# junqiangchen/PytorchDeepLearing

Hardware: AMD Instinct MI355X
Metric: volumes/sec VNet3d 96^3 fp16 train step (higher is better)
Workload: dtype f16; 1 GPU; VNet3d(1,1) binary seg, 4x1x96^3 per GPU, BinaryDiceLoss + Dice metric, AdamW, dropout p=0.2 on, random-init weights (BASELINE.json configs[2]); global_batch=4, parallelism=dp1, loss_semantics=per-rank (DDP)

## Files before the change

### include/segengine.h

```cpp
#ifndef SEGENGINE_H
#define SEGENGINE_H
#ifdef __cplusplus
extern "C" {
#endif

typedef struct seg_engine* seg_handle;

enum { SEG_NET_VNET = 0, SEG_NET_UNET = 1, SEG_NET_RESNET = 2 };
enum { SEG_F32 = 0, SEG_F16 = 1, SEG_BF16 = 2 };
enum { SEG_LABEL_U8 = 0, SEG_LABEL_I32 = 1, SEG_LABEL_I64 = 2, SEG_LABEL_F32 = 3,
       SEG_LABEL_BINARIZE = 16 };
enum {
    SEG_LOSS_BINARY_DICE = 0,
    SEG_LOSS_BINARY_CE = 1,
    SEG_LOSS_BINARY_FOCAL = 2,
    SEG_LOSS_BINARY_CE_DICE = 3,
    SEG_LOSS_MULTI_CE = 4,
    SEG_LOSS_MULTI_FOCAL = 5,
    SEG_LOSS_MULTI_DICE = 6,
    SEG_LOSS_BINARY_JACCARD = 7,
    SEG_LOSS_BINARY_ELDICE = 8,
    SEG_LOSS_BINARY_TVERSKY = 9,
    SEG_LOSS_MULTI_CE_DICE = 10,
    SEG_LOSS_MULTI_ELDICE = 11,
// ... 130 lines not shown
    int Cout, Ngemm, K, Kpad;
    int sd, sh, sw;
    int scatter;
    seg_taps taps;
    const float* act_scale;
    const float* act_shift;
    void* out1;
    int Cout0;
    const void* rq_r;
    const float* rq_scale;
    const float* rq_shift;
    double* rq_Q;
} seg_conv_args;
int seg_op_conv(const seg_conv_args* a, int dtype, void* stream);
int seg_op_conv_kernel(const seg_conv_args* a);

typedef struct seg_wgrad_args {
    const void* dr;
    const void* x0;
    const void* x1;
    int C0, C1;
    float* dw;
    int P, Q;
    int N, ID, IH, IW, OD, OH, OW;
    int sd, sh, sw;
    seg_taps taps;
    long long sP, sQ, sT;
    int stem;
    const float* act_scale;
    const float* act_shift;
} seg_wgrad_args;
long long seg_op_wgrad_partial_bytes(const seg_wgrad_args* a);
int seg_op_wgrad(const seg_wgrad_args* a, float* partial_scratch, int dtype, void* stream);

typedef struct seg_pack_desc {
    const float* src;
    void* dst;
    int R1, R2, T, Cc;
    int Kpad;
    long long s1, s2, sT, sC;
    int flipT;
    int csrc;
    int frag;
} seg_pack_desc;
int seg_op_pack(const seg_pack_desc* descs, int ndesc, long long max_elems, int dtype, void* stream);
int seg_op_conv3(const void* in, const void* w, const float* bias, void* out, double* stats, int n, int d, int h,
                 int wid, int cin, int cout, int ndim, int dtype, void* stream);
long long seg_op_wgrad3_partial_bytes(int ndim, int n, int d, int h, int wid, int p, int q);
int seg_op_wgrad3(const void* dr, const void* x, float* partial, float* dw, int n, int d, int h, int wid, int p,
                  int q, int ndim, int dtype, void* stream);
int seg_op_wgrad3_cat(const void* dr, const void* x0, const void* x1, int c0, float* partial, float* dw, int n, int d, int h,
                      int wid, int p, int q, int ndim, int dtype, void* stream);
typedef struct seg_stemx_args {
    const void* img; const void* w3; const void* w1;
    const float* bias3; const float* bias1;
    double* stats3; double* stats1;
    const float* scale3; const float* shift3; const float* scale1; const float* shift1;
    void* out;
    const void* dy[3]; int ndy;
    double* Q3; double* Q1;
    const float* coef3; const float* coef1;
    float* partial;
    int N, D, H, W, Cimg;
} seg_stemx_args;
long long seg_op_stemx_partial_bytes(int ndim, int n, int d, int h, int wid, int cimg);
long long seg_op_stemx_moment_bytes(int ndim, int n, int d, int h, int wid, int cimg);
// ... 135 lines not shown
```

### pytorchdeeplearing_amd/_capi.py

```python
import ctypes as C
import os

HERE = os.path.dirname(os.path.abspath(__file__))
LIB_PATH = os.environ.get("SEGENGINE_LIB") or os.path.join(HERE, "lib", "libsegengine.so")

NET_KIND = {"vnet": 0, "unet": 1, "resnet": 2}
DTYPE = {"f32": 0, "fp32": 0, "float32": 0, "f16": 1, "fp16": 1, "float16": 1, "bf16": 2, "bfloat16": 2}
LABEL_TYPES = {"torch.uint8": 0, "torch.int32": 1, "torch.int64": 2, "torch.float32": 3}
LOSS_KIND = {
    "BinaryDiceLoss": 0, "BinaryCrossEntropyLoss": 1, "BinaryFocalLoss": 2, "BinaryCrossEntropyDiceLoss": 3,
    "MutilCrossEntropyLoss": 4, "MutilFocalLoss": 5, "MutilDiceLoss": 6,
    "BinaryJaccardLoss": 7, "BinaryELDiceLoss": 8, "BinaryTverskyLoss": 9, "MutilCrossEntropyDiceLoss": 10, "MutilELDiceLoss": 11, "BinarySSLoss": 12,
    "MutilTverskyLoss": 13, "MutilSSLoss": 14, "MCC_Loss": 15,
}
LABEL_BINARIZE = 16
MASKS_EVAL, MASKS_GIVEN, MASKS_RANDOM = 0, 1, 2


def label_type(t, binarize=False):
    return LABEL_TYPES[str(t.dtype)] | (LABEL_BINARIZE if binarize else 0)
KERNEL_CLASSES = ["conv3", "wgrad3", "conv_generic", "wgrad_generic", "stem", "gn_act", "gn_bwd_reduce", "gn_bwd_apply", "head", "conv3_smallbox", "gn_group", "misc", "cls_head"]

_vp, _i, _ll, _f, _d = C.c_void_p, C.c_int, C.c_longlong, C.c_float, C.c_double

# ... 19 lines not shown
    "seg_backward_bucket": (_i, [_vp, C.c_double, C.POINTER(C.c_int), C.POINTER(C.c_longlong)]),
    "seg_backward_range": (_i, [_vp, _vp, _i, _i, _i, _vp]),
    "seg_backward_slice": (_i, [_vp, _vp, _i, _i, _i, _i, _vp]),
    "seg_side_wait": (_i, [_vp, _vp]),
    "seg_feature_find": (_i, [_vp, C.c_char_p, C.POINTER(_i), C.POINTER(_i)]),
    "seg_feature_read": (_i, [_vp, _i, _i, _vp, _vp]),
    "seg_gradcam_ws_bytes": (_ll, [_vp, _i]),
    "seg_gradcam": (_i, [_vp, C.POINTER(_i), _i, _vp, _vp, _vp]),
    "seg_set_loss_scale": (_i, [_vp, _f]),
    "seg_get_loss_scale": (_f, [_vp]),
    "seg_loss_ws_bytes": (_ll, [_i, _i]),
    "seg_loss_forward": (_i, [_vp, _vp, _i, _i, _i, _ll, _i, _f, _f, _vp, _vp, _vp, _vp]),
    "seg_loss_shared_doubles": (_i, []),
    "seg_loss_reduce": (_i, [_vp, _vp, _i, _i, _i, _ll, _i, _f, _f, _vp, _vp]),
    "seg_loss_finalize": (_i, [_vp, _vp, _i, _i, _i, _ll, _i, _f, _f, _vp, _i, _vp, _vp, _vp]),
    "seg_loss_backward": (_i, [_vp, _vp, _i, _i, _i, _ll, _i, _f, _f, _vp, _f, _vp, _vp]),
    "seg_lovasz_ws_bytes": (_ll, [_i, _ll]),
    "seg_lovasz_forward": (_i, [_vp, _vp, _i, _i, _i, _ll, _vp, _vp, _vp, _vp]),
    "seg_ssim_ws_bytes": (_ll, [_i, _i, _ll]),
    "seg_ssim_forward": (_i, [_vp, _vp, _i, _i, _i, _i, _i, _i, _i, _vp, _vp, _vp]),
    "seg_ssim_forward_cols": (_i, [_vp, _vp, _i, _i, _i, _i, _i, _i, _i, _vp, _vp, _vp, _vp]),
    "seg_ssim_backward": (_i, [_vp, _vp, _i, _i, _i, _i, _i, _i, _i, _vp, _vp, _i, _vp, _vp, _vp]),
    "seg_predict_mask": (_i, [_vp, _vp, _i, _i, _ll, C.c_float, _i, _vp]),
    "seg_metric": (_i, [_vp, _vp, _i, _i, _i, _ll, _vp, _vp, _vp]),
    "seg_train_step": (_i, [_vp, _vp, _vp]),
    "seg_train_graph_capture": (_i, [_vp, _vp, _vp]),
    "seg_train_graph_launch": (_i, [_vp, _vp]),
    "seg_train_graph_ready": (_i, [_vp]),
    "seg_adam_step": (_i, [_vp, _vp, _vp, _vp, _ll, _f, _f, _f, _f, _f, _i, _f, _i, _vp, _vp]),
    "seg_op_conv": (_i, [_vp, _i, _vp]),
    "seg_op_conv_kernel": (_i, [_vp]),
    "seg_op_wgrad": (_i, [_vp, _vp, _i, _vp]),
    "seg_op_wgrad_partial_bytes": (_ll, [_vp]),
    "seg_op_pack": (_i, [_vp, _i, _ll, _i, _vp]),
    "seg_op_conv3": (_i, [_vp, _vp, _vp, _vp, _vp, _i, _i, _i, _i, _i, _i, _i, _i, _vp]),
    "seg_op_conv3x": (_i, [_i, _vp, _vp, _i, _vp, _vp, _vp, _vp, _i, _i, _i, _i, _i, _i, _i, _i, _vp]),
    "seg_op_conv3x_num_cfgs": (_i, []),
    "seg_op_conv3x_cfg_info": (_i, [_i, C.POINTER(_i), C.POINTER(_i), C.POINTER(_i), C.POINTER(_i), C.POINTER(_i), C.c_char_p, _i]),
    "seg_op_conv3x_default_cfg": (_i, [_i, _i, _i, _i, _i, _i, _i, _i]),
    "seg_op_conv3x_cfg_frag": (_i, [_i]),
    "seg_op_wgrad3_partial_bytes": (_ll, [_i, _i, _i, _i, _i, _i, _i]),
    "seg_op_wgrad3": (_i, [_vp, _vp, _vp, _vp, _i, _i, _i, _i, _i, _i, _i, _i, _vp]),
    "seg_op_wgrad3_cat": (_i, [_vp, _vp, _vp, _i, _vp, _vp, _i, _i, _i, _i, _i, _i, _i, _i, _vp]),
    "seg_op_stemx_partial_bytes": (_ll, [_i, _i, _i, _i, _i, _i]),
    "seg_op_stemx_moment_bytes": (_ll, [_i, _i, _i, _i, _i, _i]),
    "seg_op_stemx": (_i, [_vp, _i, _i, _i, _vp, _vp, _vp]),
    "seg_abi_sizeof": (_i, [_i]),
    "seg_op_gn_forward": (_i, [_vp, _i, _vp]),
    "seg_op_gn_backward": (_i, [_vp, _i, _vp]),
    "seg_op_gn_backward_head": (_i, [_vp, _vp, _vp, _vp, _i, _vp]),
    "seg_op_gn_coop_plan": (_i, [_i, _ll, _i, _i, C.POINTER(_i), C.POINTER(_i)]),
    "seg_op_gn_group_eligible": (_i, [_i, _ll, _i]),
    "seg_op_maxpool": (_i, [_vp, _vp, _vp, _vp, _i, _i, _i, _i, _i, _i, _i, _i, _i, _i, _vp]),
    "seg_op_cls_head_ws_bytes": (_ll, [_i, _ll]),
    "seg_op_cls_head_ws_offset": (_ll, [_i, _ll, _i]),
    "seg_op_cls_head_forward": (_i, [_vp, _vp, _vp, _vp, _vp, _vp, _vp, _i, _ll, _i, _vp, _i, _vp]),
    "seg_op_cls_head_backward": (_i, [_vp, _vp, _vp, _vp, _vp, _vp, _vp, _vp, _i, _ll, _i, _i, _vp, _i, _vp]),
    "seg_op_gradcam_ws_bytes": (_ll, [_i, _i, _i, _i, _i, _i, _i, _i]),
    "seg_op_gradcam": (_i, [_vp, _vp, _i, _i, _i, _i, _i, _i, _i, _i, _i, _i, _f, _f, _i, _i, _vp, _vp, _vp]),
    "seg_op_pool3": (_i, [_vp, _vp, _i, _i, _i, _i, _i, _i, _vp]),
    "seg_op_skel_iter": (_i, [_vp, _vp, _vp, _i, _i, _i, _i, _i, _vp]),
    "seg_op_skel_iter_bwd": (_i, [_vp, _vp, _vp, _vp, _vp, _i, _i, _i, _i, _i, _vp]),
    "seg_op_skel_update": (_i, [_vp, _vp, _vp, _i, _i, _i, _i, _i, _vp]),
    "seg_op_skel_update_bwd": (_i, [_vp, _vp, _vp, _vp, _vp, _i, _i, _i, _i, _i, _vp]),
    "seg_op_pool3_bwd": (_i, [_vp, _vp, _vp, _i, _i, _i, _i, _i, _i, _vp]),
    "seg_op_plane_dot_scratch_bytes": (_ll, [_i, _ll]),
# ... 109 lines not shown
```

### pytorchdeeplearing_amd/csrc/capi_ops.hip

```cpp
#include <cmath>

#include "engine_internal.h"

#define SEG_OK(what) (hipGetLastError() == hipSuccess ? 0 : fail(what ": launch failed"))

extern "C" {

long long seg_loss_ws_bytes(int n, int c) { return (long long)align_up(loss_sums_count(n, c) * sizeof(double) * STAT_REP); }

}
namespace segi {
int fill_loss(LossArgs& a, const float* logits, const void* target, int label_type, int n, int c, long long v,
                     int loss_kind, float focal_alpha, float focal_gamma, void* ws) {
    if (!logits || !target || !ws) return fail("loss: null pointer");
    if (c < 1 || c > 16) return fail("loss: classes must be 1..16");
    if (loss_kind < 0 || loss_kind >= L_KIND_COUNT) return fail("loss: unknown loss kind");
    const bool binary_kind = loss_kind <= SEG_LOSS_BINARY_CE_DICE || (loss_kind >= L_BIN_JACCARD && loss_kind <= L_BIN_TVERSKY) || loss_kind == L_BIN_SS ||
                             loss_kind == L_BIN_MCC;
    if ((c == 1) != binary_kind) return fail("loss: binary losses need C == 1, multi-class losses C > 1");
    a.logits = logits; a.target = target; a.label_type = label_type; a.N = n; a.C = c; a.V = v; a.kind = loss_kind;
    a.focal_alpha = focal_alpha; a.focal_gamma = focal_gamma; a.class_alpha = nullptr; a.sums = (double*)ws;
    a.out = nullptr; a.dlogits = nullptr; a.grad_scale = 1.f; a.phase = 0; a.n_global = 0;
    return 0;
}
// ... 365 lines not shown
    return SEG_OK("seg_adam_step");
}
}
extern "C" {
int seg_adam_step(float* params, const float* grads, float* exp_avg, float* exp_avg_sq, long long numel, float lr, float beta1,
                  float beta2, float eps, float weight_decay, int decoupled, float inv_scale, int check_finite, int* state, void* stream) {
    return adam_step_impl(params, grads, exp_avg, exp_avg_sq, numel, lr, beta1, beta2, eps, weight_decay, decoupled, inv_scale, check_finite, state,
                          stream, false);
}

int seg_op_conv(const seg_conv_args* a, int dtype, void* stream) {
    if (!a || !a->in0 || !a->w || !a->out) return fail("seg_op_conv: null pointer");
    const int cin = a->C0 + a->C1;
    if (cin < 8 || (cin & (cin - 1)) || a->C0 % 8) return fail("seg_op_conv: channel counts must be powers of two >= 8");
    if (a->Cout % 16 || a->Ngemm % 16 || a->Kpad % 32 || a->Kpad < a->K) return fail("seg_op_conv: bad GEMM extents");
    if ((a->act_scale || a->act_shift) && !(a->act_scale && a->act_shift && conv_uses_stream_kernel(*a)))
        return fail("seg_op_conv: act_scale / act_shift need the streaming kernel (gather form, seg_op_conv_kernel == 1) and come as a pair");
    if (a->rq_Q && !(a->out1 && conv_uses_stream_kernel(*a))) return fail("seg_op_conv: rq_* need out1 / Cout0 on the streaming kernel and all of rq_r, rq_scale, rq_shift");
    if (a->out1 && !conv_uses_stream_kernel(*a)) return fail("seg_op_conv: out1 / Cout0 need the streaming kernel (gather form, no bias / stats, 16-channel tiles in pairs)");
    launch_conv_igemm(*a, dtype, (hipStream_t)stream);
    return SEG_OK("seg_op_conv");
}
int seg_op_conv_kernel(const seg_conv_args* a) { return a ? (conv_uses_stream_kernel(*a) ? 1 : 0) : -1; }
long long seg_op_wgrad_partial_bytes(const seg_wgrad_args* a) { return a ? (long long)wgrad_partial_bytes(*a) : -1; }
int seg_op_wgrad(const seg_wgrad_args* a, float* partial_scratch, int dtype, void* stream) {
    if (!a || !a->dr || !a->x0 || !a->dw || !partial_scratch) return fail("seg_op_wgrad: null pointer");
    if (a->P % 16) return fail("seg_op_wgrad: P must be a multiple of 16");
    if (a->stem ? (a->Q > 32) : (a->Q % 16 != 0)) return fail("seg_op_wgrad: bad Q");
    if ((a->act_scale || a->act_shift) && !(a->act_scale && a->act_shift && dtype != SEG_F32 && wgrad_act_supported(*a)))
        return fail("seg_op_wgrad: act_scale / act_shift need a 1^d stride-1 conv on 16-bit tensors with C0 <= 64 and come as a pair");
    launch_wgrad(*a, partial_scratch, dtype, (hipStream_t)stream);
    return SEG_OK("seg_op_wgrad");
}
int seg_op_pack(const seg_pack_desc* descs, int ndesc, long long max_elems, int dtype, void* stream) {
    if (!descs || ndesc < 1) return fail("seg_op_pack: no descriptors");
    launch_pack(descs, ndesc, (int)max_elems, dtype, (hipStream_t)stream);
    return SEG_OK("seg_op_pack");
}
int seg_op_conv3(const void* in, const void* w, const float* bias, void* out, double* stats, int n, int d, int h, int wid, int cin,
                 int cout, int ndim, int dtype, void* stream) {
    if (!in || !w || !out) return fail("seg_op_conv3: null pointer");
    if (cin < 16 || (cin & (cin - 1)) || cout % 16) return fail("seg_op_conv3: Cin must be a power of two >= 16, Cout a multiple of 16");
    launch_conv3(in, w, bias, out, stats, n, ndim == 3 ? d : 1, h, wid, cin, cout, ndim, dtype, (hipStream_t)stream);
    return SEG_OK("seg_op_conv3");
}
int seg_op_conv3x(int cfg, const void* in0, const void* in1, int c0, const void* w, const float* bias, void* out, double* stats, int n, int d,
                  int h, int wid, int cin, int cout, int ndim, int dtype, void* stream) {
    if (!in0 || !w || !out) return fail("seg_op_conv3x: null pointer");
    if (ndim != 2 && ndim != 3) return fail("seg_op_conv3x: ndim must be 2 or 3");
    const int dd = ndim == 3 ? d : 1;
    if (!conv3x_supported(dtype, ndim, n, dd, h, wid, cin, cout, c0, in1 != nullptr))
        return fail("seg_op_conv3x: needs a 16-bit dtype, Cin % 32 == 0 (or Cin == 16 without a concat), Cout % 16 == 0 and tensors below 2 GB per sample");
    if (cfg < 0) cfg = conv3x_pick(ndim, n, dd, h, wid, cin, cout);
    if (cfg < 0 || !launch_conv3x(cfg, in0, in1, c0, w, bias, out, stats, n, dd, h, wid, cin, cout, ndim, dtype, (hipStream_t)stream))
        return fail("seg_op_conv3x: the tiling does not fit this shape");
    return SEG_OK("seg_op_conv3x");
}
int seg_op_conv3x_num_cfgs(void) { return conv3x_num_cfgs(); }
int seg_op_conv3x_cfg_frag(int cfg) { return conv3x_cfg_frag(cfg); }
int seg_op_conv3x_cfg_info(int index, int* id, int* ndim, int* box3, int* bn, int* nres, char* name, int name_cap) {
    const char* nm = nullptr;
    if (conv3x_cfg_info(index, id, ndim, box3, bn, nres, &nm)) return fail("seg_op_conv3x_cfg_info: index out of range");
    if (name && name_cap > 0) snprintf(name, name_cap, "%s", nm);
    return 0;
}
int seg_op_conv3x_default_cfg(int ndim, int n, int d, int h, int wid, int cin, int cout, int dtype) {
// ... 303 lines not shown
```

### pytorchdeeplearing_amd/csrc/kernels.h

```cpp
#pragma once
#include "../../include/segengine.h"
#include "common.h"

namespace seg {

typedef seg_taps Taps;
typedef seg_conv_args ConvArgs;
struct StepRider { int* bump = nullptr; const int* gate = nullptr; int* tally = nullptr; int* clear = nullptr; };
__device__ __forceinline__ void step_rider_run(const StepRider& r) {
    if (r.bump) { if (!(r.gate && *r.gate)) *r.bump += 1; else if (r.tally) *r.tally += 1; }
    if (r.clear) *r.clear = 0;
}
void launch_conv_igemm(const ConvArgs& a, int dtype, hipStream_t s, int stat_rep = STAT_REP);
bool conv_uses_stream_kernel(const ConvArgs& a);

void launch_conv3(const void* in, const void* w, const float* bias, void* out, double* stats, int N, int D, int H, int W, int Cin,
                  int Cout, int ndim, int dtype, hipStream_t s, const void* in1 = nullptr, int C0 = 0);
bool conv3x_supported(int dtype, int ndim, int N, int D, int H, int W, int Cin, int Cout, int C0, bool has_in1);
int conv3x_pick(int ndim, int N, int D, int H, int W, int Cin, int Cout, bool has_in1 = false);
int conv3x_cfg_frag(int cfg);
int conv3x_num_cfgs();
int conv3x_cfg_info(int index, int* id, int* ndim, int* box3, int* bn, int* nres, const char** name);
bool launch_conv3x(int cfg, const void* in0, const void* in1, int C0, const void* w, const float* bias, void* out, double* stats, int N, int D,
                   int H, int W, int Cin, int Cout, int ndim, int dtype, hipStream_t s, int stat_rep = STAT_REP);
// ... 128 lines not shown
    const float* vdl; const float* vw; int vK;    int rep_q;
};
struct GnHeadW { double* sums; float* dw; float* db; };
bool gn_head_w_supported(const GnBwdArgs& a);
void launch_gn_bwd_reduce(const GnBwdArgs& a, int dtype, hipStream_t s, const GnHeadW* hw = nullptr);
struct GnBwdFinArgs;
void launch_gn_bwd_apply(const GnBwdArgs& a, int dtype, hipStream_t s, const GnBwdFinArgs* fa = nullptr, const GnBwdFinArgs* fb = nullptr,
                         const GnHeadW* hw = nullptr);

struct GnBwdFinArgs {
    const double* Q;
    const double* stats;
    const float* gamma;
    const float* mask; int mask_ld;
    const float* mean; const float* rstd;
    float* dgamma; float* dbeta;
    float* dbias;
    float* coef;
    int N, C;
    long long V;
    int rep_q, rep_s;
};
void launch_gn_bwd_finalize(const GnBwdFinArgs& a, hipStream_t s, const GnBwdFinArgs* b = nullptr);
bool gn_bwd_group_eligible(int C, long long V, int esz);
void launch_gn_fwd_group(const GnFinArgs& f, const void* r, const void* res, void* out, int dtype, hipStream_t s);
void launch_gn_bwd_group(const GnBwdArgs& e, const GnBwdFinArgs& f, int dtype, hipStream_t s);
bool gn_bwd_coop_plan(int C, long long V, int N, int esz, int* S, int* ku);
bool gn_bwd_coop_eligible(const GnBwdArgs& e, int esz);
void launch_gn_bwd_coop(const GnBwdArgs& e, const GnBwdFinArgs& f, int dtype, hipStream_t s);

typedef seg_wgrad_args WgradArgs;
size_t wgrad_partial_bytes(const WgradArgs& a);
void launch_wgrad(const WgradArgs& a, float* partial, int dtype, hipStream_t s, int qreal = 0);
bool wgrad_act_supported(const WgradArgs& a);

struct PoolArgs {
    const void* in; void* out;
    const void* dout; void* din;
    int N, D, H, W, C;
    int pd, ph, pw;
};
void launch_maxpool_fwd(const PoolArgs& a, int dtype, hipStream_t s);
void launch_maxpool_bwd(const PoolArgs& a, int dtype, hipStream_t s);

void launch_ingest(const float* x, void* out, int N, int C, long long V, int dtype, hipStream_t s, int Csrc = 0, StepRider rd = StepRider{});

typedef seg_pack_desc PackDesc;
void launch_pack(const PackDesc* descs_dev, int ndesc, int max_rows, int dtype, hipStream_t s, StepRider rd = StepRider{});

enum LossKind { L_BIN_DICE = 0, L_BIN_CE = 1, L_BIN_FOCAL = 2, L_BIN_CE_DICE = 3, L_MC_CE = 4, L_MC_FOCAL = 5, L_MC_DICE = 6,
                L_BIN_JACCARD = 7, L_BIN_ELDICE = 8, L_BIN_TVERSKY = 9, L_MC_CE_DICE = 10, L_MC_ELDICE = 11, L_BIN_SS = 12,
                L_MC_TVERSKY = 13, L_MC_SS = 14,
                L_BIN_MCC = 15,
                L_KIND_COUNT = 16 };
struct LossArgs {
    const float* logits;
    const void* target; int label_type;
    int N, C; long long V;
    int kind;
    float focal_alpha, focal_gamma;
    const float* class_alpha;
    double* sums;
    float* out;
    float* dlogits;
    float grad_scale;
    int phase;
// ... 110 lines not shown
```

### pytorchdeeplearing_amd/csrc/wgrad.hip

```cpp
#include "kernels.h"
#include "dispatch.h"
#include "gn_math.h"
#include <cstdlib>

namespace seg {
namespace {

constexpr int WM = 32;
constexpr int WT = 64;
constexpr int LDW = WT + 8;
constexpr int MAXTB = 8;

struct RowCoord { int n, d, h, w; };
__device__ __forceinline__ RowCoord decode_row(long long m64, int D, int H, int W) {
    int m = (int)m64;
    RowCoord r;
    r.w = m % W; m /= W;
    r.h = m % H; m /= H;
    r.d = m % D;
    r.n = m / D;
    return r;
}

template <class T> struct TFrag {
    static __device__ __forceinline__ typename Mma<T>::frag load(const T* tile, int col0, int lane) {
        const int t = lane & 15, q = lane >> 4;
        const T* p0 = tile + (4 * q + (t >> 2)) * LDW + col0 + (t & 3) * 4;
        const s16x4 lo = lds_read_tr16(p0);
        const s16x4 hi = lds_read_tr16(p0 + 16 * LDW);
        vec<short, 8> v;
#pragma unroll
        for (int j = 0; j < 4; ++j) { v[j] = lo[j]; v[4 + j] = hi[j]; }
        return __builtin_bit_cast(typename Mma<T>::frag, v);
    }
};
template <> struct TFrag<float> {
    static __device__ __forceinline__ Mma<float>::frag load(const float* tile, int col0, int lane) {
        const int t = lane & 15, q = lane >> 4;
        Mma<float>::frag f;
#pragma unroll
        for (int j = 0; j < 8; ++j) f[j] = tile[(4 * j + q) * LDW + col0 + t];
        return f;
    }
};

struct WgPlan { int TP, TQ, ntq, ntile, TB, ntg; long long Mc; int parts; int direct; };

#ifndef SEG_EMU
#define SEG_WG_WAVES(x) __attribute__((amdgpu_waves_per_eu(x)))
#else
#define SEG_WG_WAVES(x)
#endif
template <class T, bool STEM, int NTB>
__global__ __launch_bounds__(256) SEG_WG_WAVES(NTB == MAXTB && sizeof(T) == 2 ? 3 : 1) void wgrad_kernel(WgradArgs a, WgPlan pl, float* partial) {
    constexpr int WMT = (NTB == 1 && !STEM) ? 128 : WM;
    constexpr int NPC = WMT * 8 / 256;
    __shared__ T Ds[WMT * LDW];
    __shared__ T Xs[NTB * WMT * LDW];
    const int tid = threadIdx.x, lane = tid & 63, wv = tid >> 6;
    const int tg = (int)(blockIdx.x / pl.ntile), tile = (int)(blockIdx.x % pl.ntile);
    const int tap0 = tg * NTB;
    const int TP = pl.TP, TQ = pl.TQ;
    const int p0 = (tile / pl.ntq) * TP, q0 = (tile % pl.ntq) * TQ;
    const long long M = (long long)a.N * a.OD * a.OH * a.OW;
    const long long mbeg = (long long)blockIdx.y * pl.Mc;
    const long long mend = (mbeg + pl.Mc < M) ? mbeg + pl.Mc : M;
    const T* dr = (const T*)a.dr;
    const T* x0 = (const T*)a.x0;
    const T* x1 = (const T*)a.x1;
    const int ntaps = STEM ? 1 : a.taps.n;
    const int ntb = (ntaps - tap0 < NTB) ? ntaps - tap0 : NTB;

    const int nt_p = TP / 16, nt_q = (TQ + 15) / 16, n16 = nt_p * nt_q;
    const int nwork = ntb * n16;
// ... 248 lines not shown
                    }
                    store8(&Xs[xrow[u] * LDW + ((u * 256 + tid) % cpr_q) * 8], ((okq[k] >> (8 + u)) & 1u) ? xv : zero8<T>());
                }
                __syncthreads();
#pragma unroll
                for (int i = 0; i < MAXW; ++i) {
                    const int wi = wv + 4 * i;
                    if (wi < n16) {
                        const int pi = wi / nt_q, qi = wi % nt_q;
#pragma unroll
                        for (int kk = 0; kk < WMT / 32; ++kk) {
                            const typename Mma<T>::frag af = TFrag<T>::load(Ds + kk * 32 * LDW, pi * 16, lane);
                            const typename Mma<T>::frag bf = TFrag<T>::load(Xs + kk * 32 * LDW, qi * 16, lane);
                            acc[i] = Mma<T>::run(af, bf, acc[i]);
                        }
                    }
                }
                __syncthreads();
            }
        }
    }
    const int l15 = lane & 15, q = lane >> 4;
    const int Qc = a.Q;
    float* dst = partial + (long long)blockIdx.y * a.P * Qc;
#pragma unroll
    for (int i = 0; i < MAXW; ++i) {
        const int wi = wv + 4 * i;
        if (wi < n16) {
            const int pi = wi / nt_q, qi = wi % nt_q;
            const int qq = q0 + qi * 16 + l15;
#pragma unroll
            for (int r = 0; r < 4; ++r) dst[(long long)(p0 + pi * 16 + 4 * q + r) * Qc + qq] = acc[i][r];
        }
    }
}

__global__ __launch_bounds__(256) void wgrad_reduce_kernel(const float* partial, float* dw, int P, int Tn, int Qc, int parts, long long sP,
                                                           long long sQ, long long sT, int stem_cimg, int qreal) {
    const long long total = (long long)P * Tn * Qc;
    const int b0 = blockIdx.y * 32, b1 = (b0 + 32 < parts) ? b0 + 32 : parts;
    for (long long i = (long long)blockIdx.x * 256 + threadIdx.x; i < total; i += (long long)gridDim.x * 256) {
        float s0 = 0.f, s1 = 0.f, s2 = 0.f, s3 = 0.f;
        int b = b0;
        for (; b + 4 <= b1; b += 4) {
            s0 += partial[(long long)b * total + i]; s1 += partial[(long long)(b + 1) * total + i];
            s2 += partial[(long long)(b + 2) * total + i]; s3 += partial[(long long)(b + 3) * total + i];
        }
        for (; b < b1; ++b) s0 += partial[(long long)b * total + i];
        const int qq = (int)(i % Qc), tap = (int)((i / Qc) % Tn), p = (int)(i / ((long long)Qc * Tn));
        if (!stem_cimg && qq >= qreal) continue;
        long long o;
        if (stem_cimg) o = p * sP + (qq % stem_cimg) * sQ + (qq / stem_cimg) * sT;
        else o = p * sP + qq * sQ + tap * sT;
        const float tot = (s0 + s1) + (s2 + s3);
        if (gridDim.y == 1) dw[o] += tot;
        else atomicAdd(&dw[o], tot);
    }
}

WgPlan make_plan(const WgradArgs& a) {
    WgPlan pl;
    const long long M = (long long)a.N * a.OD * a.OH * a.OW;
    const int T = a.stem ? 1 : a.taps.n;
    pl.TB = (T <= MAXTB) ? T : 1;
    int cap = (pl.TB > 1) ? 32 : WT;
    pl.TP = a.P < cap ? a.P : cap;
    if (a.stem) { pl.TQ = 32; pl.ntq = 1; }
    else { pl.TQ = a.Q < cap ? a.Q : cap; pl.ntq = a.Q / pl.TQ; }
    pl.ntile = (a.P / pl.TP) * pl.ntq;
    pl.ntg = (T + pl.TB - 1) / pl.TB;
    const int bx = pl.ntg * pl.ntile;
    constexpr long long total = 2048;
    constexpr long long pcap = 4ll << 20;
    long long parts = total / bx;
    if (parts < 1) parts = 1;
    if (parts > 1024) parts = 1024;
    const long long elems = (long long)a.P * T * a.Q;
    if (parts * elems > pcap) parts = pcap / elems;
    if (parts < 1) parts = 1;
    const long long maxp = (M + WM - 1) / WM;
    if (parts > maxp) parts = maxp;
    const int step = (pl.TB == 1 && !a.stem) ? 128 : WM;
    long long Mc = (M + parts - 1) / parts;
    Mc = (Mc + step - 1) / step * step;
    pl.Mc = Mc;
    pl.direct = (!a.stem && T == 1 && a.sd == 1 && a.sh == 1 && a.sw == 1 && a.taps.d[0] == 0 && a.taps.h[0] == 0 && a.taps.w[0] == 0 &&
                 a.ID == a.OD && a.IH == a.OH && a.IW == a.OW) ? 1 : 0;
    pl.parts = (int)((M + Mc - 1) / Mc);
    return pl;
}

template <class T>
void wgrad_dispatch(const WgradArgs& a, float* partial, hipStream_t s, int qreal) {
    const WgPlan pl = make_plan(a);
    dim3 grid(pl.ntg * pl.ntile, pl.parts);
    static const bool direct_on = (knob_i("SEG_WG_DIRECT", 1) != 0);
    bool done = false;
    if constexpr (sizeof(T) == 2) {
        if ((direct_on || a.act_scale) && !a.stem && pl.TB == 1 && pl.direct && pl.ntg == 1 && a.C0 % 8 == 0) {
            const int np = pl.TP % 16 ? 0 : pl.TP / 16, nq = pl.TQ % 16 ? 0 : pl.TQ / 16;
            done = by_int<124, 243, 443, 114, 224>(100 * np + 10 * nq + (nq == 4 ? 3 : 4), [&](auto k) { by_bool(a.act_scale != nullptr, [&](auto act) {
                hipLaunchKernelGGL(HIP_KERNEL_NAME(wgrad_direct_kernel<T, k() / 100, k() / 10 % 10, k() % 10, act()>), grid, dim3(256), 0, s, a, pl, partial);
            }); });
        }
    }
    if (a.act_scale && !done) { fprintf(stderr, "segengine: activation on load needs the direct weight-gradient kernel (internal error)\n"); abort(); }
    if (done) {}
    else if (a.stem) hipLaunchKernelGGL(HIP_KERNEL_NAME(wgrad_kernel<T, true, 1>), grid, dim3(256), 0, s, a, pl, partial);
    else if (pl.TB == 1) hipLaunchKernelGGL(HIP_KERNEL_NAME(wgrad_kernel<T, false, 1>), grid, dim3(256), 0, s, a, pl, partial);
    else hipLaunchKernelGGL(HIP_KERNEL_NAME(wgrad_kernel<T, false, MAXTB>), grid, dim3(256), 0, s, a, pl, partial);
    const int Tn = a.stem ? 1 : a.taps.n;
    const long long total = (long long)a.P * Tn * a.Q;
    int blocks = (int)((total + 255) / 256);
    if (blocks > 4096) blocks = 4096;
    hipLaunchKernelGGL(wgrad_reduce_kernel, dim3(blocks, (pl.parts + 31) / 32), dim3(256), 0, s, (const float*)partial, a.dw, a.P, Tn, a.Q, pl.parts, a.sP, a.sQ,
                       a.sT, a.stem ? a.C0 : 0, (qreal > 0 && qreal < a.Q) ? qreal : a.Q);
}

}

bool wgrad_act_supported(const WgradArgs& a) {
    if (a.stem || a.C0 % 8 || a.C0 > 64) return false;
    const WgPlan pl = make_plan(a);
    if (!(pl.TB == 1 && pl.direct && pl.ntg == 1)) return false;
    if (pl.Mc > (long long)a.OD * a.OH * a.OW && a.N > 2) return false;
    const int np = pl.TP / 16, nq = pl.TQ / 16;
    return pl.TP % 16 == 0 && pl.TQ % 16 == 0 &&
           ((np == 1 && nq == 2) || (np == 2 && nq == 4) || (np == 4 && nq == 4) || (np == 1 && nq == 1) || (np == 2 && nq == 2));
}

size_t wgrad_partial_bytes(const WgradArgs& a) {
    const WgPlan pl = make_plan(a);
    return (size_t)pl.parts * a.P * (a.stem ? 1 : a.taps.n) * a.Q * sizeof(float);
}

void launch_wgrad(const WgradArgs& a, float* partial, int dtype, hipStream_t s, int qreal) {
    by_dtype(dtype, [&](auto t) { wgrad_dispatch<tag_type<decltype(t)>>(a, partial, s, qreal); });
}

}
```

### pytorchdeeplearing_amd/ops.py

```python
import ctypes as C

import torch

from . import _capi
from .engine import aligned_empty

TORCH_DTYPE = {"f32": torch.float32, "f16": torch.float16, "bf16": torch.bfloat16}


class Taps(C.Structure):
    _fields_ = [("n", C.c_int), ("d", C.c_byte * 27), ("h", C.c_byte * 27), ("w", C.c_byte * 27)]


class ConvArgs(C.Structure):
    _fields_ = [("in0", C.c_void_p), ("in1", C.c_void_p), ("C0", C.c_int), ("C1", C.c_int), ("w", C.c_void_p),
                ("bias", C.c_void_p), ("out", C.c_void_p), ("stats", C.c_void_p),
                ("N", C.c_int), ("ID", C.c_int), ("IH", C.c_int), ("IW", C.c_int),
                ("OD", C.c_int), ("OH", C.c_int), ("OW", C.c_int),
                ("FD", C.c_int), ("FH", C.c_int), ("FW", C.c_int),
                ("Cout", C.c_int), ("Ngemm", C.c_int), ("K", C.c_int), ("Kpad", C.c_int),
                ("sd", C.c_int), ("sh", C.c_int), ("sw", C.c_int), ("scatter", C.c_int), ("taps", Taps),
                ("act_scale", C.c_void_p), ("act_shift", C.c_void_p), ("out1", C.c_void_p), ("Cout0", C.c_int),
                ("rq_r", C.c_void_p), ("rq_scale", C.c_void_p), ("rq_shift", C.c_void_p), ("rq_Q", C.c_void_p)]

# ... 174 lines not shown
        oshape = (N, a.FD, a.FH, a.FW, cout)
    else:
        a.scatter = 0
        od = (D + 2 * pad - k) // stride + 1 if ndim == 3 else 1
        a.OD, a.OH, a.OW = od, (H + 2 * pad - k) // stride + 1, (W + 2 * pad - k) // stride + 1
        a.sd, a.sh, a.sw = (stride if ndim == 3 else 1), stride, stride
        a.taps = make_taps(ndim, k, pad)
        a.K, a.Ngemm = a.taps.n * cin, cout
        oshape = (N, a.OD, a.OH, a.OW, cout)
    a.Kpad = _kpad(a.K)
    assert tuple(wpacked.shape) == (a.Ngemm, a.Kpad), (tuple(wpacked.shape), a.Ngemm, a.Kpad)
    out = _alloc(oshape if not split else oshape[:-1] + (split,), TORCH_DTYPE[dtype], x0.device, zero=True)
    a.out = out.data_ptr()
    out1 = None
    if split:
        out1 = _alloc(oshape[:-1] + (cout - split,), TORCH_DTYPE[dtype], x0.device, zero=True)
        a.out1, a.Cout0 = out1.data_ptr(), split
    q = None
    if rq is not None:
        q = _alloc((32, N, split, 2), torch.float64, x0.device, zero=True)
        a.rq_r, a.rq_scale, a.rq_shift, a.rq_Q = rq[0].data_ptr(), rq[1].data_ptr(), rq[2].data_ptr(), q.data_ptr()
    stats = None
    if want_stats:
        stats = _alloc((32, N, cout, 2), torch.float64, x0.device, zero=True)
        a.stats = stats.data_ptr()
    global last_conv_kernel
    last_conv_kernel = lib.dll.seg_op_conv_kernel(C.byref(a))
    lib.check(lib.dll.seg_op_conv(C.byref(a), _capi.DTYPE[dtype], _capi.stream_for(x0.device)), "seg_op_conv")
    if split:
        return (out, out1, q.sum(0)) if q is not None else (out, out1)
    return (out, stats.sum(0)) if want_stats else out


def wgrad(dr, x0, dtype, ndim, k, stride=1, pad=0, x1=None, stem=False, act=None):
    lib = _capi.lib_for(dr.device)
    N, OD, OH, OW, P = dr.shape
    _, D, H, W, C0 = x0.shape
    a = WgradArgs()
    a.dr, a.x0, a.C0 = dr.data_ptr(), x0.data_ptr(), C0
    a.x1, a.C1 = (x1.data_ptr(), x1.shape[-1]) if x1 is not None else (None, 0)
    a.taps = make_taps(ndim, k, pad)
    T = a.taps.n
    qc = C0 + a.C1
    a.P, a.Q = P, (T * qc if stem else qc)
    a.N, a.ID, a.IH, a.IW, a.OD, a.OH, a.OW = N, D, H, W, OD, OH, OW
    a.sd, a.sh, a.sw = (stride if ndim == 3 else 1), stride, stride
    a.sP, a.sQ, a.sT = qc * T, T, 1
    a.stem = 1 if stem else 0
    if act is not None:
        a.act_scale, a.act_shift = act[0].data_ptr(), act[1].data_ptr()
    dw = _alloc((P, qc) + (k,) * ndim, torch.float32, dr.device, zero=True)
    a.dw = dw.data_ptr()
    scratch = aligned_empty(lib.seg_op_wgrad_partial_bytes(C.byref(a)), dr.device)
    lib.check(lib.seg_op_wgrad(C.byref(a), scratch.data_ptr(), _capi.DTYPE[dtype], _capi.stream_for(dr.device)), "seg_op_wgrad")
    return dw


def conv3(x, wpacked, dtype, ndim, cout, bias=None, want_stats=False, out=None):
    lib = _capi.lib_for(x.device)
    N, D, H, W, cin = x.shape
    if out is None:
        out = _alloc((N, D, H, W, cout), TORCH_DTYPE[dtype], x.device, zero=True)
    stats = _alloc((32, N, cout, 2), torch.float64, x.device, zero=True) if want_stats else None
    lib.check(lib.seg_op_conv3(x.data_ptr(), wpacked.data_ptr(), bias.data_ptr() if bias is not None else None, out.data_ptr(),
                               stats.data_ptr() if stats is not None else None, N, D, H, W, cin, cout, ndim, _capi.DTYPE[dtype],
                               _capi.stream_for(x.device)), "seg_op_conv3")
    return (out, stats.sum(0)) if want_stats else out


def wgrad3(dr, x, dtype, ndim, x1=None):
    lib = _capi.lib_for(dr.device)
    N, D, H, W, P = dr.shape
    Q = x.shape[-1] + (x1.shape[-1] if x1 is not None else 0)
    if x1 is not None:
        nbytes = lib.seg_op_wgrad3_partial_bytes(ndim, N, D, H, W, P, Q)
        partial = aligned_empty(nbytes, dr.device).view(torch.float32)
        dw = _alloc((P, Q) + (3,) * ndim, torch.float32, dr.device, zero=True)
        lib.check(lib.seg_op_wgrad3_cat(dr.data_ptr(), x.data_ptr(), x1.data_ptr(), x.shape[-1], partial.data_ptr(), dw.data_ptr(), N, D, H, W,
                                        P, Q, ndim, _capi.DTYPE[dtype], _capi.stream_for(dr.device)), "seg_op_wgrad3_cat")
        return dw
    nbytes = lib.seg_op_wgrad3_partial_bytes(ndim, N, D, H, W, P, Q)
    partial = aligned_empty(nbytes, dr.device).view(torch.float32)
    dw = _alloc((P, Q) + (3,) * ndim, torch.float32, dr.device, zero=True)
    lib.check(lib.seg_op_wgrad3(dr.data_ptr(), x.data_ptr(), partial.data_ptr(), dw.data_ptr(), N, D, H, W, P, Q, ndim,
                                _capi.DTYPE[dtype], _capi.stream_for(dr.device)), "seg_op_wgrad3")
    return dw


# ... 234 lines not shown
```

Measured before the change: 1082 volumes/s.

## Add specialized stride-2 weight-gradient kernel for 2x2 downsampling convs with 16 input channels

Adds a dedicated wgrad kernel for stride-2, kernel-2 convolutions (8 or 4 taps) with 16 input channels. It software-pipelines global loads into registers over a configurable depth, stages tiles in LDS and runs MFMA over 128-row M chunks. A new plan sizes the split-M partition so each workgroup gets a minimum number of steps. This is meant to cut the overhead of the generic direct/tiled path on the VNet down-convolutions, at the cost of more kernel variants and a different partial-sum layout. Debug hooks (kernel id query, partial buffer return) are added too.

New measurement: 1096 volumes/s (median of 6 runs). 1.01x the previous value.

```diff
diff --git a/include/segengine.h b/include/segengine.h
--- a/include/segengine.h
+++ b/include/segengine.h
@@ -186,6 +186,7 @@
 } seg_wgrad_args;
 long long seg_op_wgrad_partial_bytes(const seg_wgrad_args* a);
 int seg_op_wgrad(const seg_wgrad_args* a, float* partial_scratch, int dtype, void* stream);
+int seg_op_wgrad_kernel(const seg_wgrad_args* a, int dtype);
 
 typedef struct seg_pack_desc {
     const float* src;
diff --git a/pytorchdeeplearing_amd/_capi.py b/pytorchdeeplearing_amd/_capi.py
--- a/pytorchdeeplearing_amd/_capi.py
+++ b/pytorchdeeplearing_amd/_capi.py
@@ -75,6 +75,7 @@
     "seg_op_conv_kernel": (_i, [_vp]),
     "seg_op_wgrad": (_i, [_vp, _vp, _i, _vp]),
     "seg_op_wgrad_partial_bytes": (_ll, [_vp]),
+    "seg_op_wgrad_kernel": (_i, [_vp, _i]),
     "seg_op_pack": (_i, [_vp, _i, _ll, _i, _vp]),
     "seg_op_conv3": (_i, [_vp, _vp, _vp, _vp, _vp, _i, _i, _i, _i, _i, _i, _i, _i, _vp]),
     "seg_op_conv3x": (_i, [_i, _vp, _vp, _i, _vp, _vp, _vp, _vp, _i, _i, _i, _i, _i, _i, _i, _i, _vp]),
diff --git a/pytorchdeeplearing_amd/csrc/capi_ops.hip b/pytorchdeeplearing_amd/csrc/capi_ops.hip
--- a/pytorchdeeplearing_amd/csrc/capi_ops.hip
+++ b/pytorchdeeplearing_amd/csrc/capi_ops.hip
@@ -421,6 +421,7 @@
     launch_wgrad(*a, partial_scratch, dtype, (hipStream_t)stream);
     return SEG_OK("seg_op_wgrad");
 }
+int seg_op_wgrad_kernel(const seg_wgrad_args* a, int dtype) { return a ? wgrad_kernel_id(*a, dtype) : -1; }
 int seg_op_pack(const seg_pack_desc* descs, int ndesc, long long max_elems, int dtype, void* stream) {
     if (!descs || ndesc < 1) return fail("seg_op_pack: no descriptors");
     launch_pack(descs, ndesc, (int)max_elems, dtype, (hipStream_t)stream);
diff --git a/pytorchdeeplearing_amd/csrc/kernels.h b/pytorchdeeplearing_amd/csrc/kernels.h
--- a/pytorchdeeplearing_amd/csrc/kernels.h
+++ b/pytorchdeeplearing_amd/csrc/kernels.h
@@ -184,6 +184,7 @@
 typedef seg_wgrad_args WgradArgs;
 size_t wgrad_partial_bytes(const WgradArgs& a);
 void launch_wgrad(const WgradArgs& a, float* partial, int dtype, hipStream_t s, int qreal = 0);
+int wgrad_kernel_id(const WgradArgs& a, int dtype);
 bool wgrad_act_supported(const WgradArgs& a);
 
 struct PoolArgs {
diff --git a/pytorchdeeplearing_amd/csrc/wgrad.hip b/pytorchdeeplearing_amd/csrc/wgrad.hip
--- a/pytorchdeeplearing_amd/csrc/wgrad.hip
+++ b/pytorchdeeplearing_amd/csrc/wgrad.hip
@@ -22,24 +22,24 @@
     return r;
 }
 
-template <class T> struct TFrag {
+template <class T, int LD = LDW> struct TFrag {
     static __device__ __forceinline__ typename Mma<T>::frag load(const T* tile, int col0, int lane) {
         const int t = lane & 15, q = lane >> 4;
-        const T* p0 = tile + (4 * q + (t >> 2)) * LDW + col0 + (t & 3) * 4;
+        const T* p0 = tile + (4 * q + (t >> 2)) * LD + col0 + (t & 3) * 4;
         const s16x4 lo = lds_read_tr16(p0);
-        const s16x4 hi = lds_read_tr16(p0 + 16 * LDW);
+        const s16x4 hi = lds_read_tr16(p0 + 16 * LD);
         vec<short, 8> v;
 #pragma unroll
         for (int j = 0; j < 4; ++j) { v[j] = lo[j]; v[4 + j] = hi[j]; }
         return __builtin_bit_cast(typename Mma<T>::frag, v);
     }
 };
-template <> struct TFrag<float> {
+template <int LD> struct TFrag<float, LD> {
     static __device__ __forceinline__ Mma<float>::frag load(const float* tile, int col0, int lane) {
         const int t = lane & 15, q = lane >> 4;
         Mma<float>::frag f;
 #pragma unroll
-        for (int j = 0; j < 8; ++j) f[j] = tile[(4 * j + q) * LDW + col0 + t];
+        for (int j = 0; j < 8; ++j) f[j] = tile[(4 * j + q) * LD + col0 + t];
         return f;
     }
 };
@@ -354,6 +354,103 @@
 #pragma unroll
             for (int r = 0; r < 4; ++r) dst[(long long)(p0 + pi * 16 + 4 * q + r) * Qc + qq] = acc[i][r];
         }
+    }
+}
+
+#ifndef SEG_WG_S2_DEPTH
+#define SEG_WG_S2_DEPTH 2
+#endif
+template <class T, int NT, int DEPTH, bool CHAIN>
+__global__ __launch_bounds__(256) void wgrad_s2_kernel(WgradArgs a, WgPlan pl, float* partial) {
+    constexpr int WMT = 128, TP = 32, TQ = 16, LDD = TP + 8, LDX = TQ + 8;
+    constexpr int NG = NT / 2;
+    constexpr int MAXW = NT / 2;
+    __shared__ T Ds[WMT * LDD];
+    __shared__ T Xs[NT * WMT * LDX];
+    const int tid = threadIdx.x, lane = tid & 63, wv = tid >> 6;
+    const int p0 = (int)blockIdx.x * TP;
+    const int M = a.N * a.OD * a.OH * a.OW;
+    const int mbeg = (int)((long long)blockIdx.y * pl.Mc);
+    const int mend = (mbeg + pl.Mc < M) ? (int)(mbeg + pl.Mc) : M;
+    f32x4 acc[MAXW];
+#pragma unroll
+    for (int i = 0; i < MAXW; ++i) acc[i] = f32x4{0.f, 0.f, 0.f, 0.f};
+    const int r0 = tid >> 2, c = tid & 3;
+    const T* dbase = (const T*)a.dr + p0 + c * 8;
+    const T* xbase = (const T*)a.x0 + c * 8;
+    long long goff[NG];
+#pragma unroll
+    for (int g = 0; g < NG; ++g) goff[g] = ((long long)a.taps.d[2 * g] * a.IH + a.taps.h[2 * g]) * a.IW * TQ;
+    int OD = a.OD, OH = a.OH, OW = a.OW;
+    settle(OD); settle(OH); settle(OW);
+    vec<T, 8> dq[DEPTH][2], xq[DEPTH][NG][2];
+    unsigned okq[DEPTH];
+    auto issue = [&](int slot, int ms) {
+        const T* dsrc[2];
+        const T* xsrc[2];
+        unsigned ok = 0u;
+#pragma unroll
+        for (int u = 0; u < 2; ++u) {
+            const int m = ms + r0 + 64 * u;
+            const bool v = m < mend;
+            ok |= v ? (1u << u) : 0u;
+            const int mc = v ? m : mbeg;
+            const RowCoord r = decode_row(mc, OD, OH, OW);
+            const long long vox = (((long long)r.n * a.ID + r.d * a.sd) * a.IH + r.h * a.sh) * a.IW + r.w * a.sw;
+            dsrc[u] = dbase + (long long)mc * a.P;
+            xsrc[u] = xbase + vox * TQ;
+        }
+        okq[slot] = ok;
+        __builtin_amdgcn_sched_barrier(0);
+#pragma unroll
+        for (int u = 0; u < 2; ++u) {
+            dq[slot][u] = load8(dsrc[u]);
+#pragma unroll
+            for (int g = 0; g < NG; ++g) xq[slot][g][u] = load8(xsrc[u] + goff[g]);
+        }
+        __builtin_amdgcn_sched_barrier(0);
+    };
+#pragma unroll
+    for (int k = 0; k < DEPTH - 1; ++k) issue(k, mbeg + k * WMT);
+    for (int ms = mbeg; ms < mend; ms += DEPTH * WMT) {
+#pragma unroll
+        for (int k = 0; k < DEPTH; ++k) {
+            issue((k + DEPTH - 1) % DEPTH, ms + (k + DEPTH - 1) * WMT);
+#pragma unroll
+            for (int u = 0; u < 2; ++u) {
+                const bool v = (okq[k] >> u) & 1u;
+                const int row = r0 + 64 * u;
+                store8(&Ds[row * LDD + c * 8], v ? dq[k][u] : zero8<T>());
+#pragma unroll
+                for (int g = 0; g < NG; ++g) store8(&Xs[((2 * g + (c >> 1)) * WMT + row) * LDX + (c & 1) * 8], v ? xq[k][g][u] : zero8<T>());
+            }
+            __syncthreads();
+            const int pi = wv & 1, tb = (wv >> 1) * MAXW;
+            f32x4 part[CHAIN ? 1 : MAXW][CHAIN ? 1 : WMT / 32];
+#pragma unroll
+            for (int kk = 0; kk < WMT / 32; ++kk) {
+                const typename Mma<T>::frag af = TFrag<T, LDD>::load(Ds + kk * 32 * LDD, pi * 16, lane);
+#pragma unroll
+                for (int i = 0; i < MAXW; ++i) {
+                    const typename Mma<T>::frag bf = TFrag<T, LDX>::load(Xs + ((tb + i) * WMT + kk * 32) * LDX, 0, lane);
+                    if constexpr (CHAIN) acc[i] = Mma<T>::run(af, bf, acc[i]);
+                    else part[i][kk] = Mma<T>::run(af, bf, f32x4{0.f, 0.f, 0.f, 0.f});
+                }
+            }
+            if constexpr (!CHAIN) {
+#pragma unroll
+                for (int i = 0; i < MAXW; ++i) acc[i] += (part[i][0] + part[i][1]) + (part[i][2] + part[i][3]);
+            }
+            __syncthreads();
+        }
+    }
+    const int l15 = lane & 15, q = lane >> 4;
+    const int pi = wv & 1, tb = (wv >> 1) * MAXW;
+    float* dst = partial + (long long)blockIdx.y * a.P * NT * TQ;
+#pragma unroll
+    for (int i = 0; i < MAXW; ++i) {
+#pragma unroll
+        for (int r = 0; r < 4; ++r) dst[((long long)(p0 + pi * 16 + 4 * q + r) * NT + tb + i) * TQ + l15] = acc[i][r];
     }
 }
 
@@ -412,16 +509,68 @@
     return pl;
 }
 
+#ifndef SEG_WG_S2_WGS
+#define SEG_WG_S2_WGS 512
+#endif
+#ifndef SEG_WG_S2_MINSTEPS
+#define SEG_WG_S2_MINSTEPS 7
+#endif
+bool wgrad_s2_eligible(const WgradArgs& a, int elem_size) {
+    if (elem_size != 2 || a.stem || a.act_scale || a.act_shift || a.x1 || a.C1) return false;
+    const int T = a.taps.n;
+    if (T != 8 && T != 4) return false;
+    const bool d3 = T == 8;
+    for (int t = 0; t < T; ++t)
+        if (a.taps.d[t] != (d3 ? t >> 2 : 0) || a.taps.h[t] != ((t >> 1) & 1) || a.taps.w[t] != (t & 1)) return false;
+    if (a.sd != (d3 ? 2 : 1) || a.sh != 2 || a.sw != 2) return false;
+    if (d3 ? a.ID != 2 * a.OD : (a.ID != 1 || a.OD != 1)) return false;
+    if (a.IH != 2 * a.OH || a.IW != 2 * a.OW) return false;
+    if (a.P % 32 || a.Q != 16 || a.C0 != 16) return false;
+    const long long fine = (long long)a.N * a.ID * a.IH * a.IW;
+    return a.N > 0 && a.OD > 0 && a.OH > 0 && a.OW > 0 && fine < (1ll << 31) - (1 << 16);
+}
+int wgrad_s2_mode() { return knob_i("SEG_WG_S2", 1); }
+WgPlan wgrad_s2_plan(const WgradArgs& a, WgPlan base, int mode) {
+    base.ntile = a.P / 32; base.ntq = 1; base.ntg = 1;
+    if (mode == 2) return base;
+    const long long M = (long long)a.N * a.OD * a.OH * a.OW;
+    long long wgs = SEG_WG_S2_WGS / base.ntile;
+    if (wgs < 1) wgs = 1;
+    long long steps = (M + 128 * wgs - 1) / (128 * wgs);
+    if (steps < SEG_WG_S2_MINSTEPS) steps = SEG_WG_S2_MINSTEPS;
+    long long parts = (M + 128 * steps - 1) / (128 * steps);
+    if (parts > base.parts) parts = base.parts;
+    base.Mc = (M + parts - 1) / parts;
+    base.parts = (int)((M + base.Mc - 1) / base.Mc);
+    return base;
+}
+bool wgrad_direct_on() {
+    static const bool on = (knob_i("SEG_WG_DIRECT", 1) != 0);
+    return on;
+}
+int wgrad_direct_key(const WgradArgs& a, const WgPlan& pl, int elem_size) {
+    if (elem_size != 2 || !(wgrad_direct_on() || a.act_scale) || a.stem || pl.TB != 1 || !pl.direct || pl.ntg != 1 || a.C0 % 8) return 0;
+    const int np = pl.TP % 16 ? 0 : pl.TP / 16, nq = pl.TQ % 16 ? 0 : pl.TQ / 16;
+    const int key = 100 * np + 10 * nq + (nq == 4 ? 3 : 4);
+    return (key == 124 || key == 243 || key == 443 || key == 114 || key == 224) ? key : 0;
+}
+
 template <class T>
 void wgrad_dispatch(const WgradArgs& a, float* partial, hipStream_t s, int qreal) {
-    const WgPlan pl = make_plan(a);
+    WgPlan pl = make_plan(a);
     dim3 grid(pl.ntg * pl.ntile, pl.parts);
-    static const bool direct_on = (knob_i("SEG_WG_DIRECT", 1) != 0);
     bool done = false;
     if constexpr (sizeof(T) == 2) {
-        if ((direct_on || a.act_scale) && !a.stem && pl.TB == 1 && pl.direct && pl.ntg == 1 && a.C0 % 8 == 0) {
-            const int np = pl.TP % 16 ? 0 : pl.TP / 16, nq = pl.TQ % 16 ? 0 : pl.TQ / 16;
-            done = by_int<124, 243, 443, 114, 224>(100 * np + 10 * nq + (nq == 4 ? 3 : 4), [&](auto k) { by_bool(a.act_scale != nullptr, [&](auto act) {
+        const int s2 = wgrad_s2_mode();
+        if (s2 && wgrad_s2_eligible(a, sizeof(T))) {
+            pl = wgrad_s2_plan(a, pl, s2);
+            grid = dim3(pl.ntile, pl.parts);
+            by_int<8, 4>(a.taps.n, [&](auto nt) { by_bool(s2 == 2, [&](auto chain) {
+                hipLaunchKernelGGL(HIP_KERNEL_NAME(wgrad_s2_kernel<T, nt(), SEG_WG_S2_DEPTH, chain()>), grid, dim3(256), 0, s, a, pl, partial);
+            }); });
+            done = true;
+        } else if (const int key = wgrad_direct_key(a, pl, sizeof(T))) {
+            done = by_int<124, 243, 443, 114, 224>(key, [&](auto k) { by_bool(a.act_scale != nullptr, [&](auto act) {
                 hipLaunchKernelGGL(HIP_KERNEL_NAME(wgrad_direct_kernel<T, k() / 100, k() / 10 % 10, k() % 10, act()>), grid, dim3(256), 0, s, a, pl, partial);
             }); });
         }
@@ -456,6 +605,12 @@
     return (size_t)pl.parts * a.P * (a.stem ? 1 : a.taps.n) * a.Q * sizeof(float);
 }
 
+int wgrad_kernel_id(const WgradArgs& a, int dtype) {
+    const int es = dtype == DT_F32 ? 4 : 2;
+    if (wgrad_s2_mode() && wgrad_s2_eligible(a, es)) return 2;
+    return wgrad_direct_key(a, make_plan(a), es) ? 1 : 0;
+}
+
 void launch_wgrad(const WgradArgs& a, float* partial, int dtype, hipStream_t s, int qreal) {
     by_dtype(dtype, [&](auto t) { wgrad_dispatch<tag_type<decltype(t)>>(a, partial, s, qreal); });
 }
diff --git a/pytorchdeeplearing_amd/ops.py b/pytorchdeeplearing_amd/ops.py
--- a/pytorchdeeplearing_amd/ops.py
+++ b/pytorchdeeplearing_amd/ops.py
@@ -230,7 +230,10 @@
     return (out, stats.sum(0)) if want_stats else out
 
 
-def wgrad(dr, x0, dtype, ndim, k, stride=1, pad=0, x1=None, stem=False, act=None):
+last_wgrad_kernel = None
+
+
+def wgrad(dr, x0, dtype, ndim, k, stride=1, pad=0, x1=None, stem=False, act=None, with_partial=False):
     lib = _capi.lib_for(dr.device)
     N, OD, OH, OW, P = dr.shape
     _, D, H, W, C0 = x0.shape
@@ -250,8 +253,12 @@
     dw = _alloc((P, qc) + (k,) * ndim, torch.float32, dr.device, zero=True)
     a.dw = dw.data_ptr()
     scratch = aligned_empty(lib.seg_op_wgrad_partial_bytes(C.byref(a)), dr.device)
+    if with_partial:
+        scratch.view(torch.float32).fill_(float("nan"))
+    global last_wgrad_kernel
+    last_wgrad_kernel = lib.seg_op_wgrad_kernel(C.byref(a), _capi.DTYPE[dtype])
     lib.check(lib.seg_op_wgrad(C.byref(a), scratch.data_ptr(), _capi.DTYPE[dtype], _capi.stream_for(dr.device)), "seg_op_wgrad")
-    return dw
+    return (dw, scratch.view(torch.float32)) if with_partial else dw
 
 
 def conv3(x, wpacked, dtype, ndim, cout, bias=None, want_stats=False, out=None):
```
